# pranshu-raj-211/dmdqn

Hardware: NVIDIA B200
Metric: agent-updates/sec (higher is better)
Workload: dtype f32

## Files before the change

dmdqn_b200/csrc/learn_tc.cu:

```cuda
#include <cuda.h>
#include <string.h>
#include "common.cuh"

namespace dmdqn {

namespace {

constexpr int H = 256;
constexpr int BM = 128;
constexpr int EW = 16;
constexpr int NT = EW * 32;
constexpr int W_MMA = EW, W_TMA = EW + 1, W_CONV = EW + 2;
constexpr int CONV_WARPS = 6, CONV_GROUP_WARPS = 2;
constexpr int NT_F = (EW + 8) * 32;
constexpr int REGS_EPI = 104, REGS_AUX = 32;
constexpr int KC = 16;
constexpr uint32_t ATOM = BM * 128;
constexpr unsigned long long WAIT_LIMIT_NS = 2000000000ull;

__device__ __forceinline__ uint32_t smem_u32(const void* p) { return (uint32_t)__cvta_generic_to_shared(p); }

__device__ __forceinline__ uint64_t make_desc(uint32_t saddr, uint32_t lbo_bytes, uint32_t sbo_bytes, uint32_t layout) {
    return (uint64_t)((saddr >> 4) & 0x3FFF) | (uint64_t)((lbo_bytes >> 4) & 0x3FFF) << 16 |
           (uint64_t)((sbo_bytes >> 4) & 0x3FFF) << 32 | (uint64_t)1 << 46 | (uint64_t)layout << 61;
// ... 59 lines not shown
template <int N> __device__ __forceinline__ void regs_inc() { asm volatile("setmaxnreg.inc.sync.aligned.u32 %0;" ::"n"(N)); }
template <int N> __device__ __forceinline__ void regs_dec() { asm volatile("setmaxnreg.dec.sync.aligned.u32 %0;" ::"n"(N)); }
__device__ __forceinline__ void epi_sync() { asm volatile("bar.sync 1, 512;" ::: "memory"); }
__device__ __forceinline__ void l2_prefetch(const void* p, uint32_t bytes) {
    asm volatile("cp.async.bulk.prefetch.L2.global [%0], %1;" ::"l"(p), "r"(bytes) : "memory");
}
__device__ __forceinline__ void fence_async_smem() { asm volatile("fence.proxy.async.shared::cta;" ::: "memory"); }
__device__ __forceinline__ void tc_fence_before() { asm volatile("tcgen05.fence::before_thread_sync;" ::: "memory"); }
__device__ __forceinline__ void tc_fence_after() { asm volatile("tcgen05.fence::after_thread_sync;" ::: "memory"); }

__device__ __forceinline__ void tmem_ld32(uint32_t taddr, float (&v)[32]) {
    uint32_t r[32];
    asm volatile(
        "tcgen05.ld.sync.aligned.32x32b.x32.b32 {%0,%1,%2,%3,%4,%5,%6,%7,%8,%9,%10,%11,%12,%13,%14,%15,%16,%17,%18,%19,%20,%21,"
        "%22,%23,%24,%25,%26,%27,%28,%29,%30,%31}, [%32];\n"
        : "=r"(r[0]), "=r"(r[1]), "=r"(r[2]), "=r"(r[3]), "=r"(r[4]), "=r"(r[5]), "=r"(r[6]), "=r"(r[7]), "=r"(r[8]),
          "=r"(r[9]), "=r"(r[10]), "=r"(r[11]), "=r"(r[12]), "=r"(r[13]), "=r"(r[14]), "=r"(r[15]), "=r"(r[16]),
          "=r"(r[17]), "=r"(r[18]), "=r"(r[19]), "=r"(r[20]), "=r"(r[21]), "=r"(r[22]), "=r"(r[23]), "=r"(r[24]),
          "=r"(r[25]), "=r"(r[26]), "=r"(r[27]), "=r"(r[28]), "=r"(r[29]), "=r"(r[30]), "=r"(r[31])
        : "r"(taddr));
    asm volatile("tcgen05.wait::ld.sync.aligned;" ::: "memory");
#pragma unroll
    for (int j = 0; j < 32; ++j) v[j] = __uint_as_float(r[j]);
}
__device__ __forceinline__ void tmem_st32(uint32_t taddr, const float (&v)[32]) {
    asm volatile(
        "tcgen05.st.sync.aligned.32x32b.x32.b32 [%0], {%1,%2,%3,%4,%5,%6,%7,%8,%9,%10,%11,%12,%13,%14,%15,%16,%17,%18,%19,%20,"
        "%21,%22,%23,%24,%25,%26,%27,%28,%29,%30,%31,%32};\n" ::"r"(taddr),
        "r"(__float_as_uint(v[0])), "r"(__float_as_uint(v[1])), "r"(__float_as_uint(v[2])), "r"(__float_as_uint(v[3])),
        "r"(__float_as_uint(v[4])), "r"(__float_as_uint(v[5])), "r"(__float_as_uint(v[6])), "r"(__float_as_uint(v[7])),
        "r"(__float_as_uint(v[8])), "r"(__float_as_uint(v[9])), "r"(__float_as_uint(v[10])), "r"(__float_as_uint(v[11])),
        "r"(__float_as_uint(v[12])), "r"(__float_as_uint(v[13])), "r"(__float_as_uint(v[14])), "r"(__float_as_uint(v[15])),
        "r"(__float_as_uint(v[16])), "r"(__float_as_uint(v[17])), "r"(__float_as_uint(v[18])), "r"(__float_as_uint(v[19])),
        "r"(__float_as_uint(v[20])), "r"(__float_as_uint(v[21])), "r"(__float_as_uint(v[22])), "r"(__float_as_uint(v[23])),
        "r"(__float_as_uint(v[24])), "r"(__float_as_uint(v[25])), "r"(__float_as_uint(v[26])), "r"(__float_as_uint(v[27])),
        "r"(__float_as_uint(v[28])), "r"(__float_as_uint(v[29])), "r"(__float_as_uint(v[30])), "r"(__float_as_uint(v[31]))
        : "memory");
}
__device__ __forceinline__ void tmem_st_wait() { asm volatile("tcgen05.wait::st.sync.aligned;" ::: "memory"); }

__device__ __forceinline__ float tf32_hi(float x) {
    return __uint_as_float((__float_as_uint(x) + 0x1000u) & 0xffffe000u);
}
template <int PASSES>
__device__ __forceinline__ void split4(const float4& x, float4& hi, float4& lo) {
    if (PASSES == 1) { hi = x; lo = make_float4(0.f, 0.f, 0.f, 0.f); return; }
    hi = make_float4(tf32_hi(x.x), tf32_hi(x.y), tf32_hi(x.z), tf32_hi(x.w));
    lo = make_float4(x.x - hi.x, x.y - hi.y, x.z - hi.z, x.w - hi.w);
}

__device__ __forceinline__ uint32_t off_k128(int rows, int r, int k) {
    return (uint32_t)((k >> 5) * rows * 128 + r * 128 + ((((k & 31) >> 2) ^ (r & 7)) << 4) + ((k & 3) << 2));
}
__device__ __forceinline__ uint32_t off_mn(int mn_total, int k, int mn) {
    return (uint32_t)((k >> 2) * (mn_total >> 5) * 512 + (mn >> 5) * 512 + (k & 3) * 128 +
                      ((((mn & 31) >> 3) ^ (k & 3)) << 5) + ((mn & 7) << 2));
}

__device__ __forceinline__ void flag_release_add(int* f) {
    asm volatile("red.release.gpu.global.add.s32 [%0], 1;" ::"l"(f) : "memory");
}
__device__ __forceinline__ bool flag_acquire_ge(const int* f, int want) {
    for (int i = 0; i < (1 << 21); ++i) {
        int v;
        asm volatile("ld.acquire.gpu.global.s32 %0, [%1];" : "=r"(v) : "l"(f) : "memory");
        if (v >= want) return true;
        __nanosleep(256);
    }
    return false;
}
#ifdef TC_TIMING
__device__ __forceinline__ unsigned smid_() { unsigned r; asm volatile("mov.u32 %0, %%smid;" : "=r"(r)); return r; }
#endif
__device__ __forceinline__ void pdl_launch_dependents() { asm volatile("griddepcontrol.launch_dependents;" ::: "memory"); }

#ifdef TC_TIMING
#define KT_BEGIN const long long kt0_ = clock64(); long long kt1_ = 0
#define KT_END(name) do { if (threadIdx.x == 0 && (blockIdx.x % 37 == 0 || blockIdx.x == gridDim.x - 1)) \
        printf("%s cta %d kernel total %lld cycles, first item at %lld\n", name, blockIdx.x, clock64() - kt0_, kt1_ - kt0_); } while (0)
#define KT_FIRST() do { if (!kt1_) kt1_ = clock64(); } while (0)
#define TS_DECL long long ts_[16]; int tsi_ = 0
#define TS() do { if (tsi_ < 16) ts_[tsi_++] = clock64(); } while (0)
#define TS_D(i) (i < tsi_ ? ts_[i] - ts_[i - 1] : 0LL)
#define TS_PRINT(name) do { if (TC_TIMING > 1 && threadIdx.x == 0 && (blockIdx.x == 0 || blockIdx.x == 77 || blockIdx.x == gridDim.x - 1)) \
        printf("%s cta %d: %lld %lld %lld %lld %lld %lld %lld %lld %lld %lld %lld %lld | total %lld\n", name, blockIdx.x, TS_D(1), TS_D(2), TS_D(3), \
               TS_D(4), TS_D(5), TS_D(6), TS_D(7), TS_D(8), TS_D(9), TS_D(10), TS_D(11), TS_D(12), ts_[tsi_ - 1] - ts_[0]); tsi_ = 0; } while (0)
#define WG_TS_DECL long long wts_[20]; int wtsi_ = 0
#define WG_TS() do { if (wtsi_ < 20) wts_[wtsi_++] = clock64(); } while (0)
#define WG_D(i) ((i) < wtsi_ ? wts_[i] - wts_[(i) - 1] : 0LL)
#define WG_TS_PRINT(name, cond) do { if (TC_TIMING > 1 && (cond) && (blockIdx.x == 0 || blockIdx.x == 100)) \
        printf("%s cta %d: %lld %lld %lld %lld %lld %lld %lld %lld %lld %lld %lld %lld %lld %lld\n", name, blockIdx.x, WG_D(1), WG_D(2), WG_D(3), WG_D(4), \
               WG_D(5), WG_D(6), WG_D(7), WG_D(8), WG_D(9), WG_D(10), WG_D(11), WG_D(12), WG_D(13), WG_D(14)); } while (0)
#else
#define KT_FIRST()
#define KT_BEGIN
#define KT_END(name)
#define TS_DECL
#define TS()
#define TS_PRINT(name)
#define WG_TS_DECL
#define WG_TS()
#define WG_TS_PRINT(name, cond)
#endif

struct Fwd {
    static constexpr uint32_t R = 0;
    static constexpr uint32_t XLO = 3 * ATOM;
    static constexpr uint32_t WB = 8 * ATOM;
    static constexpr uint32_t BIAS1 = WB + 81920;
    static constexpr uint32_t BIAS2 = BIAS1 + 1024;
    static constexpr uint32_t W3S = BIAS2 + 1024;
    static constexpr uint32_t QP = W3S + 4096;
    static constexpr uint32_t ROWF = QP + 8192;
    static constexpr uint32_t BARS = ROWF + 3840;
    static constexpr uint32_t TOTAL = ROWF + 4096;
};
struct Bar {
    static constexpr uint32_t TMA_B = 112, CONV_B = 152, EMPTY_B = 192;
    static constexpr uint32_t AREADY = 232, DONE = 240;
    static constexpr uint32_t TMEM = 248;
};
constexpr int NSB = 5;
constexpr uint32_t STG_B = 16384, RAW_B = 8192;

struct Ring {
    uint32_t b = 0, gemms = 0;
};

__device__ __forceinline__ float4 ldg_stream(const float* p) {
    float4 v;
    asm volatile("ld.global.nc.L1::no_allocate.v4.f32 {%0,%1,%2,%3}, [%4];" : "=f"(v.x), "=f"(v.y), "=f"(v.z), "=f"(v.w) : "l"(p));
    return v;
}
__device__ __forceinline__ float4 ldg_plain(const float* p) {
    float4 v;
    asm volatile("ld.global.cg.v4.f32 {%0,%1,%2,%3}, [%4];" : "=f"(v.x), "=f"(v.y), "=f"(v.z), "=f"(v.w) : "l"(p));
    return v;
}
__device__ __forceinline__ void sts4(uint32_t a, const float4& v) {
    asm volatile("st.shared.v4.f32 [%0], {%1,%2,%3,%4};" ::"r"(a), "f"(v.x), "f"(v.y), "f"(v.z), "f"(v.w) : "memory");
}
__device__ __forceinline__ float4 lds4(uint32_t a) {
    float4 v;
    asm volatile("ld.shared.v4.f32 {%0,%1,%2,%3}, [%4];" : "=f"(v.x), "=f"(v.y), "=f"(v.z), "=f"(v.w) : "r"(a));
    return v;
}

constexpr int PF = 6;
__device__ __forceinline__ bool tma_fwd(uint32_t sbase, const CUtensorMap* tm, int g, const float* __restrict__ W, int K, Ring& r,
                                            bool ok, const float* __restrict__ next) {
    const uint32_t bars = sbase + Fwd::BARS;
    const int nchunks = K >> 3;
    for (int c = 0; c < nchunks; ++c) {
        const uint32_t s = r.b % NSB, u = r.b / NSB;
        if (c + PF < nchunks) l2_prefetch(W + (size_t)(c + PF) * 8 * H, RAW_B);
        else if (next) l2_prefetch(next + (size_t)(c + PF - nchunks) * 8 * H, RAW_B);
        if (u && ok) ok = mbar_wait(bars + Bar::EMPTY_B + 8 * s, (u - 1) & 1);
        mbar_expect_tx(bars + Bar::TMA_B + 8 * s, RAW_B);
        tma_load_5d(sbase + Fwd::WB + s * STG_B, tm, 0, 0, 0, 2 * c, g, bars + Bar::TMA_B + 8 * s);
        ++r.b;
    }
    return ok;
}
__device__ __forceinline__ bool tma_bwd(uint32_t sbase, const CUtensorMap* tm, int g, Ring& r, bool ok) {
    const uint32_t bars = sbase + Fwd::BARS;
    for (int c = 0; c < H / 8; ++c) {
        const uint32_t s = r.b % NSB, u = r.b / NSB;
        if (u && ok) ok = mbar_wait(bars + Bar::EMPTY_B + 8 * s, (u - 1) & 1);
        mbar_expect_tx(bars + Bar::TMA_B + 8 * s, RAW_B);
        tma_load_3d(sbase + Fwd::WB + s * STG_B, tm, c * 8, 0, g, bars + Bar::TMA_B + 8 * s);
        ++r.b;
    }
    return ok;
}
template <int PASSES>
__device__ __forceinline__ bool conv_ring(uint32_t sbase, int grp, int t, Ring& r, bool ok, int nchunks = H / 8) {
    const uint32_t bars = sbase + Fwd::BARS;
    constexpr int NGRP = CONV_WARPS / CONV_GROUP_WARPS;
    for (int c = 0; c < nchunks; ++c) {
        const uint32_t b = r.b + (uint32_t)c;
        if ((int)(b % NGRP) != grp) continue;
        const uint32_t s = b % NSB, u = b / NSB;
        const uint32_t st = sbase + Fwd::WB + s * STG_B;
        if (u && ok) ok = mbar_wait(bars + Bar::CONV_B + 8 * s, (u - 1) & 1);
        if (ok) ok = mbar_wait(bars + Bar::TMA_B + 8 * s, u & 1);
#pragma unroll
        for (int half = 0; half < 2; ++half) {
            float4 x[4];
#pragma unroll
            for (int i = 0; i < 4; ++i) x[i] = lds4(st + (uint32_t)(t + 64 * (4 * half + i)) * 16u);
#pragma unroll
            for (int i = 0; i < 4; ++i) {
                float4 hi, lo;
                split4<PASSES>(x[i], hi, lo);
                const uint32_t o = st + (uint32_t)(t + 64 * (4 * half + i)) * 16u;
                if (PASSES == 3) { sts4(o, hi); sts4(o + RAW_B, lo); }
            }
        }
        fence_async_smem();
        __syncwarp();
        if ((threadIdx.x & 31) == 0) mbar_arrive(bars + Bar::CONV_B + 8 * s);
    }
    r.b += (uint32_t)nchunks;
    return ok;
}

template <int PASSES, bool BT>
__device__ __forceinline__ bool mma_gemm(uint32_t sbase, uint32_t tmem, uint32_t a_hi, uint32_t a_lo_smem, uint32_t a_lo_tmem,
                                         int K, Ring& r, bool ok) {
    const uint32_t bars = sbase + Fwd::BARS;
    constexpr int KCX = 8;
    constexpr uint32_t idesc = make_idesc(false, !BT);
    const uint64_t a_hi0 = make_desc(a_hi, 16, 1024, 2);
    const uint64_t a_lo0 = make_desc(a_lo_smem, 16, 1024, 2);
    const uint64_t b0 = BT ? make_desc(sbase + Fwd::WB, 16, 256, 6) : make_desc(sbase + Fwd::WB, 512, 4096, 1);
    if (ok) ok = mbar_wait(bars + Bar::AREADY, r.gemms & 1);
    tc_fence_after();
    const int nchunks = K / KCX;
    for (int c = 0; c < nchunks; ++c) {
        const uint32_t s = r.b % NSB, u = r.b / NSB;
        if (ok) ok = mbar_wait(bars + Bar::CONV_B + 8 * s, u & 1);
        tc_fence_after();
#pragma unroll
        for (int ks = 0; ks < KCX / 8; ++ks) {
            const int kg = c * KCX + ks * 8;
            const uint32_t a_off = ((uint32_t)(kg >> 5) * ATOM + (uint32_t)((kg & 31) >> 3) * 32) >> 4;
            const uint32_t b_off = (s * STG_B) >> 4;
            const uint64_t a_hi_d = a_hi0 + a_off;
            const uint64_t b_hi = b0 + b_off, b_lo = b0 + b_off + (RAW_B >> 4);
            uint32_t acc = (c | ks) ? 1u : 0u;
            if (PASSES == 3) {
                if (a_lo_smem) mma_ss(tmem, a_lo0 + a_off, b_hi, idesc, acc);
                else mma_ts(tmem, a_lo_tmem + (uint32_t)kg, b_hi, idesc, acc);
                mma_ss(tmem, a_hi_d, b_lo, idesc, 1u);
                acc = 1u;
            }
            mma_ss(tmem, a_hi_d, b_hi, idesc, acc);
        }
        umma_commit(bars + Bar::EMPTY_B + 8 * s);
        ++r.b;
    }
    umma_commit(bars + Bar::DONE);
    r.gemms += 1;
    return ok;
}

__device__ __forceinline__ void a_ready(uint32_t sbase) {
    fence_async_smem();
    tc_fence_before();
    __syncwarp();
    if ((threadIdx.x & 31) == 0) mbar_arrive(sbase + Fwd::BARS + Bar::AREADY);
}
__device__ __forceinline__ bool wait_gemm(uint32_t sbase, Ring& r, bool ok) {
    if (ok) ok = mbar_wait(sbase + Fwd::BARS + Bar::DONE, r.gemms & 1);
    tc_fence_after();
    r.gemms += 1;
    return ok;
}

template <int PASSES>
struct XGather {
    static constexpr int MAXP = BM * 96 / 4 / NT;
    float4 x[MAXP];
    uint32_t off[MAXP];
    int n;
    float4 sp;

    __device__ __forceinline__ void begin(const float* __restrict__ ring, const int32_t* __restrict__ rows, int r0, int B, int Dp,
                                          const float* __restrict__ P, const float* __restrict__ W3, const Layout& L) {
        {
            const int j = threadIdx.x;
            if (j < H) { sp.x = __ldg(P + L.b1 + j); sp.y = __ldg(P + L.b2 + j); }
            else sp = __ldg(reinterpret_cast<const float4*>(W3) + (j - H));
        }
        const int q = Dp >> 2;
        n = BM * q / NT;
        const int dr = NT / q, dp = NT % q;
        int r = threadIdx.x / q, pc = threadIdx.x % q;
        int32_t rid[MAXP], col[MAXP];
#pragma unroll
        for (int j = 0; j < MAXP; ++j) {
            rid[j] = -1;
            if (j < n) {
                if (r0 + r < B) rid[j] = __ldg(rows + r0 + r);
                off[j] = off_k128(BM, r, pc << 2);
                col[j] = pc << 2;
                r += dr; pc += dp;
                if (pc >= q) { pc -= q; r += 1; }
            }
        }
#pragma unroll
        for (int j = 0; j < MAXP; ++j) {
            x[j] = make_float4(0.f, 0.f, 0.f, 0.f);
            if (j < n && rid[j] >= 0) x[j] = ldg_stream(ring + (size_t)rid[j] * Dp + col[j]);
        }
    }
    __device__ __forceinline__ void store(uint32_t sbase) {
        {
            float* s = reinterpret_cast<float*>(__cvta_shared_to_generic((size_t)sbase));
            const int j = threadIdx.x;
            if (j < H) { s[Fwd::BIAS1 / 4 + j] = sp.x; s[Fwd::BIAS2 / 4 + j] = sp.y; }
            else reinterpret_cast<float4*>(s + Fwd::W3S / 4)[j - H] = sp;
        }
#pragma unroll
        for (int j = 0; j < MAXP; ++j) {
            if (j < n) {
                float4 hi, lo;
                split4<PASSES>(x[j], hi, lo);
                sts4(sbase + Fwd::R + off[j], hi);
                if (PASSES == 3) sts4(sbase + Fwd::XLO + off[j], lo);
            }
        }
    }
};

struct Epi {
    int row, part;
    uint32_t lane_addr;
    __device__ __forceinline__ Epi() {
        const int warp = threadIdx.x >> 5, lane = threadIdx.x & 31;
        row = (warp & 3) * 32 + lane;
        part = warp >> 2;
        lane_addr = (uint32_t)((warp & 3) * 32) << 16;
    }
};

template <int PASSES>
__device__ __forceinline__ void epi_hidden(uint32_t sbase, uint32_t tmem, const Epi& e, uint32_t bias_off,
                                           float* __restrict__ gout_t, int ldt, uint32_t (&mask)[2]) {
#pragma unroll 1
    for (int cc = 0; cc < 2; ++cc) {
        const int c0 = e.part * 64 + cc * 32;
        float v[32], lo[32];
        float4 bq[8];
#pragma unroll
        for (int j = 0; j < 8; ++j)
            bq[j] = lds4(sbase + bias_off + (uint32_t)(c0 + 4 * j) * 4);
        tmem_ld32(tmem + e.lane_addr + (uint32_t)c0, v);
        uint32_t m = 0;
#pragma unroll
        for (int j = 0; j < 32; j += 4) {
            const float4 b = bq[j >> 2];
            float4 x = make_float4(fmaxf(v[j] + b.x, 0.f), fmaxf(v[j + 1] + b.y, 0.f), fmaxf(v[j + 2] + b.z, 0.f),
                                   fmaxf(v[j + 3] + b.w, 0.f));
            m |= (x.x > 0.f ? 1u : 0u) << j | (x.y > 0.f ? 1u : 0u) << (j + 1) | (x.z > 0.f ? 1u : 0u) << (j + 2) |
                 (x.w > 0.f ? 1u : 0u) << (j + 3);
            if (gout_t) {
                gout_t[(size_t)(c0 + j) * ldt] = x.x; gout_t[(size_t)(c0 + j + 1) * ldt] = x.y;
                gout_t[(size_t)(c0 + j + 2) * ldt] = x.z; gout_t[(size_t)(c0 + j + 3) * ldt] = x.w;
            }
            float4 hi, l4;
            split4<PASSES>(x, hi, l4);
            sts4(sbase + Fwd::R + off_k128(BM, e.row, c0 + j), hi);
            lo[j] = l4.x; lo[j + 1] = l4.y; lo[j + 2] = l4.z; lo[j + 3] = l4.w;
        }
        mask[cc] = m;
        if (PASSES == 3) tmem_st32(tmem + e.lane_addr + 256u + (uint32_t)c0, lo);
    }
    if (PASSES == 3) tmem_st_wait();
}

__device__ __forceinline__ void epi_head(uint32_t sbase, uint32_t tmem, const Epi& e, bool keep_h2,
                                         uint32_t (&mask)[2], float (&q)[4], const float* __restrict__ b3) {
    float4 acc = make_float4(0.f, 0.f, 0.f, 0.f);
#pragma unroll 1
    for (int cc = 0; cc < 2; ++cc) {
        const int c0 = e.part * 64 + cc * 32;
        float v[32];
        tmem_ld32(tmem + e.lane_addr + (uint32_t)c0, v);
        uint32_t m = 0;
#pragma unroll
        for (int j = 0; j < 32; ++j) {
            float b;
            asm volatile("ld.shared.f32 %0, [%1];" : "=f"(b) : "r"(sbase + Fwd::BIAS2 + (uint32_t)(c0 + j) * 4));
            const float x = fmaxf(v[j] + b, 0.f);
            v[j] = x;
            m |= (x > 0.f ? 1u : 0u) << j;
            const float4 w = lds4(sbase + Fwd::W3S + (uint32_t)(c0 + j) * 16);
            acc.x = fmaf(x, w.x, acc.x); acc.y = fmaf(x, w.y, acc.y);
            acc.z = fmaf(x, w.z, acc.z); acc.w = fmaf(x, w.w, acc.w);
        }
        mask[cc] = m;
        if (keep_h2) {
#pragma unroll
            for (int j = 0; j < 32; j += 4)
                sts4(sbase + Fwd::R + off_k128(BM, e.row, c0 + j), make_float4(v[j], v[j + 1], v[j + 2], v[j + 3]));
        }
    }
    float4* qp = reinterpret_cast<float4*>(__cvta_shared_to_generic((size_t)(sbase + Fwd::QP)));
    qp[e.part * BM + e.row] = acc;
    epi_sync();
    const float4 p0 = qp[e.row], p1 = qp[BM + e.row], p2 = qp[2 * BM + e.row], p3 = qp[3 * BM + e.row];
    q[0] = ((p0.x + p1.x) + (p2.x + p3.x)) + __ldg(b3 + 0); q[1] = ((p0.y + p1.y) + (p2.y + p3.y)) + __ldg(b3 + 1);
    q[2] = ((p0.z + p1.z) + (p2.z + p3.z)) + __ldg(b3 + 2); q[3] = ((p0.w + p1.w) + (p2.w + p3.w)) + __ldg(b3 + 3);
}

__device__ __forceinline__ uint32_t tc_prologue(uint32_t sbase) {
    const int warp = threadIdx.x >> 5;
    const uint32_t bars = sbase + Fwd::BARS;
    if (threadIdx.x == 0) {
        for (int b = 0; b < NSB; ++b) {
            mbar_init(bars + Bar::TMA_B + 8 * b, 1);
            mbar_init(bars + Bar::CONV_B + 8 * b, CONV_GROUP_WARPS);
            mbar_init(bars + Bar::EMPTY_B + 8 * b, 1);
        }
        mbar_init(bars + Bar::AREADY, EW);
        mbar_init(bars + Bar::DONE, 1);
        asm volatile("fence.mbarrier_init.release.cluster;" ::: "memory");
    }
    if (warp == 0) {
        asm volatile("tcgen05.alloc.cta_group::1.sync.aligned.shared::cta.b32 [%0], %1;" ::"r"(bars + Bar::TMEM), "r"(512));
        asm volatile("tcgen05.relinquish_alloc_permit.cta_group::1.sync.aligned;" ::);
    }
    tc_fence_before();
    __syncthreads();
    tc_fence_after();
    uint32_t tmem;
    asm volatile("ld.shared.u32 %0, [%1];" : "=r"(tmem) : "r"(bars + Bar::TMEM));
    return tmem;
}
__device__ __forceinline__ void tc_epilogue(uint32_t tmem) {
    tc_fence_before();
    __syncthreads();
    if ((threadIdx.x >> 5) == 0) asm volatile("tcgen05.dealloc.cta_group::1.sync.aligned.b32 %0, %1;" ::"r"(tmem), "r"(512));
}

template <bool DUELING>
__device__ __forceinline__ const float* head_w3(const LearnArgs& A, const float* P, int tgt, int g) {
    if constexpr (DUELING) return (tgt ? A.head[1] : A.head[0]) + (size_t)g * A.head_stride;
    else return P + A.L.w3;
}
template <bool DUELING>
__device__ __forceinline__ const float* head_b3(const LearnArgs& A, const float* P, int tgt, int g) {
    if constexpr (DUELING) return head_w3<true>(A, P, tgt, g) + 4 * H;
    else return P + A.L.b3;
}

__device__ __forceinline__ int k3_next(const LearnArgs& A, int q, int n_items) {
    while (q < n_items && !A.active[(q >> 1) / A.tc_tiles]) q += gridDim.x;
    return q;
}

template <int PASSES, bool DUELING>
__global__ void __launch_bounds__(NT_F, 1) tc_target_kernel(const LearnArgs A, const __grid_constant__ CUtensorMap tm_w1,
                                                            const __grid_constant__ CUtensorMap tm_w2,
                                                            const __grid_constant__ CUtensorMap tm_w1t,
                                                            const __grid_constant__ CUtensorMap tm_w2t) {
    extern __shared__ uint8_t smem_raw[];
    const uint32_t sbase = (smem_u32(smem_raw) + 1023u) & ~1023u;
    const int B = A.d.batch, Dp = A.d.obs_stride;
    const int n_items = 2 * A.d.n_nets * A.tc_tiles;
    const int warp = threadIdx.x >> 5;
    KT_BEGIN;
    const uint32_t tmem = tc_prologue(sbase);
    if (A.chain) {
        asm volatile("griddepcontrol.wait;" ::: "memory");
        pdl_launch_dependents();
    }
    Ring ring;
    bool ok = true;
    if (warp >= EW) {
        regs_dec<REGS_AUX>();
      if (warp == W_MMA) {
        if ((threadIdx.x & 31) == 0) {
            int prev = -1;
            for (int q = k3_next(A, blockIdx.x, n_items); q < n_items; q = k3_next(A, q + gridDim.x, n_items)) {
                ok = mma_gemm<PASSES, false>(sbase, tmem, sbase + Fwd::R, sbase + Fwd::XLO, 0, Dp, ring, ok);
                if (prev >= 0) flag_release_add(A.k3_done + (size_t)((prev >> 1) / A.tc_tiles) * A.ws_tiles + (prev >> 1) % A.tc_tiles);
                prev = q;
                ok = mma_gemm<PASSES, false>(sbase, tmem, sbase + Fwd::R, 0, tmem + 256u, H, ring, ok);
            }
            if (!ok) atomicExch(A.error, 13);
        }
        __syncwarp();
      } else if (warp == W_TMA) {
        if ((threadIdx.x & 31) == 0) {
            for (int q = k3_next(A, blockIdx.x, n_items); q < n_items;) {
                const int g = (q >> 1) / A.tc_tiles;
                const float* P = ((q & 1) ? A.nets.theta_tgt : A.nets.theta) + (size_t)g * A.L.stride;
                const int qn = k3_next(A, q + gridDim.x, n_items);
                const float* Pn = qn < n_items ? ((qn & 1) ? A.nets.theta_tgt : A.nets.theta) + (size_t)((qn >> 1) / A.tc_tiles) * A.L.stride + A.L.w1 : nullptr;
                ok = tma_fwd(sbase, (q & 1) ? &tm_w1t : &tm_w1, g, P + A.L.w1, Dp, ring, ok, P + A.L.w2);
                ok = tma_fwd(sbase, (q & 1) ? &tm_w2t : &tm_w2, g, P + A.L.w2, H, ring, ok, Pn);
                q = qn;
            }
            if (!ok) atomicExch(A.error, 23);
        }
        __syncwarp();
      } else if (warp < W_CONV + CONV_WARPS) {
        const int tc = threadIdx.x - W_CONV * 32, cg = (warp - W_CONV) / CONV_GROUP_WARPS, t = tc % (CONV_GROUP_WARPS * 32);
        for (int q = k3_next(A, blockIdx.x, n_items); q < n_items; q = k3_next(A, q + gridDim.x, n_items)) {
            ok = conv_ring<PASSES>(sbase, cg, t, ring, ok, Dp / 8);
            ok = conv_ring<PASSES>(sbase, cg, t, ring, ok, H / 8);
        }
        if (!ok && tc == 0) atomicExch(A.error, 33);
      }
    } else {
        regs_inc<REGS_EPI>();
        const Epi e;
        XGather<PASSES> xg;
        int q = k3_next(A, blockIdx.x, n_items);
        if (q < n_items) {
            const int g = (q >> 1) / A.tc_tiles, rt = (q >> 1) % A.tc_tiles;
            const float* P = ((q & 1) ? A.nets.theta_tgt : A.nets.theta) + (size_t)g * A.L.stride;
            xg.begin(A.rp.next_obs, A.nrows + (size_t)g * B, rt * BM, B, Dp, P, head_w3<DUELING>(A, P, q & 1, g), A.L);
        }
        int q_last = -1;
        while (q < n_items) {
            const int item = q >> 1, pass = q & 1;
            const int g = item / A.tc_tiles, rt = item % A.tc_tiles, r0 = rt * BM;
            const float* P = (pass == 0 ? A.nets.theta : A.nets.theta_tgt) + (size_t)g * A.L.stride;
            TS_DECL;
            TS();
            KT_FIRST();
            xg.store(sbase);
            a_ready(sbase);
            epi_sync();
            TS();
            ok = wait_gemm(sbase, ring, ok);
            TS();
            uint32_t mask[2];
            epi_hidden<PASSES>(sbase, tmem, e, Fwd::BIAS1, nullptr, 0, mask);
            a_ready(sbase);
            TS();
            const int qn = k3_next(A, q + gridDim.x, n_items);
            if (qn < n_items) {
                const int gn = (qn >> 1) / A.tc_tiles, rtn = (qn >> 1) % A.tc_tiles;
                const float* Pn = ((qn & 1) ? A.nets.theta_tgt : A.nets.theta) + (size_t)gn * A.L.stride;
                xg.begin(A.rp.next_obs, A.nrows + (size_t)gn * B, rtn * BM, B, Dp, Pn, head_w3<DUELING>(A, Pn, qn & 1, gn), A.L);
            }
            ok = wait_gemm(sbase, ring, ok);
            TS();
            float qv[4];
            epi_head(sbase, tmem, e, false, mask, qv, head_b3<DUELING>(A, P, pass, g));
            TS();
            TS_PRINT("K3 store L1 epi1 L2 epi2");
            const int gr = r0 + e.row;
            if (e.part == 0 && gr < B) {
                float* out = (pass == 0 ? A.q_next : A.tq_all) + ((size_t)g * B + gr) * 4;
                *reinterpret_cast<float4*>(out) = make_float4(qv[0], qv[1], qv[2], qv[3]);
            }
            q_last = q;
            q = qn;
        }
        epi_sync();
        if (q_last >= 0 && threadIdx.x == 0) flag_release_add(A.k3_done + (size_t)((q_last >> 1) / A.tc_tiles) * A.ws_tiles + (q_last >> 1) % A.tc_tiles);
        if (!ok && threadIdx.x == 0) atomicExch(A.error, 3);
        KT_END("K3");
    }
    tc_epilogue(tmem);
}

__device__ __forceinline__ int k4_next(const LearnArgs& A, int q, int n_items) {
    while (q < n_items && !A.active[q / A.tc_tiles]) q += gridDim.x;
    return q;
}

template <int PASSES, bool DUELING>
__global__ void __launch_bounds__(NT_F, 1) tc_online_kernel(const LearnArgs A, const __grid_constant__ CUtensorMap tmap_w2,
                                                            const __grid_constant__ CUtensorMap tm_w1,
                                                            const __grid_constant__ CUtensorMap tm_w2) {
    extern __shared__ uint8_t smem_raw[];
    const uint32_t sbase = (smem_u32(smem_raw) + 1023u) & ~1023u;
    float* sf = reinterpret_cast<float*>(__cvta_shared_to_generic((size_t)sbase));
    const int B = A.d.batch, Dp = A.d.obs_stride;
    const int n_items = A.d.n_nets * A.tc_tiles;
    const int warp = threadIdx.x >> 5;
    KT_BEGIN;
    const uint32_t tmem = tc_prologue(sbase);
    if (A.chain) pdl_launch_dependents();
    Ring ring;
    bool ok = true;
    if (warp >= EW) {
        regs_dec<REGS_AUX>();
      if (warp == W_MMA) {
        if ((threadIdx.x & 31) == 0) {
            int prev = -1;
            for (int q = k4_next(A, blockIdx.x, n_items); q < n_items; q = k4_next(A, q + gridDim.x, n_items)) {
                ok = mma_gemm<PASSES, false>(sbase, tmem, sbase + Fwd::R, sbase + Fwd::XLO, 0, Dp, ring, ok);
                ok = mma_gemm<PASSES, false>(sbase, tmem, sbase + Fwd::R, 0, tmem + 256u, H, ring, ok);
                if (prev >= 0) flag_release_add(A.k4a_done + prev / A.tc_tiles);
                prev = q;
                ok = mma_gemm<PASSES, true>(sbase, tmem, sbase + Fwd::R, 0, tmem + 256u, H, ring, ok);
            }
            if (!ok) atomicExch(A.error, 14);
        }
        __syncwarp();
      } else if (warp == W_TMA) {
        if ((threadIdx.x & 31) == 0) {
            for (int q = k4_next(A, blockIdx.x, n_items); q < n_items; q = k4_next(A, q + gridDim.x, n_items)) {
                const int g = q / A.tc_tiles;
                if (A.chain && ok) ok = flag_acquire_ge(A.k3_done + (size_t)g * A.ws_tiles + q % A.tc_tiles, 2);
                const float* P = A.nets.theta + (size_t)g * A.L.stride;
                const int qn = k4_next(A, q + gridDim.x, n_items);
                const float* Pn = qn < n_items ? A.nets.theta + (size_t)(qn / A.tc_tiles) * A.L.stride + A.L.w1 : nullptr;
                ok = tma_fwd(sbase, &tm_w1, g, P + A.L.w1, Dp, ring, ok, P + A.L.w2);
                ok = tma_fwd(sbase, &tm_w2, g, P + A.L.w2, H, ring, ok, Pn);
                ok = tma_bwd(sbase, &tmap_w2, g, ring, ok);
            }
            if (!ok) atomicExch(A.error, 24);
        }
        __syncwarp();
      } else if (warp < W_CONV + CONV_WARPS) {
        const int tc = threadIdx.x - W_CONV * 32, cg = (warp - W_CONV) / CONV_GROUP_WARPS, t = tc % (CONV_GROUP_WARPS * 32);
        for (int q = k4_next(A, blockIdx.x, n_items); q < n_items; q = k4_next(A, q + gridDim.x, n_items)) {
            ok = conv_ring<PASSES>(sbase, cg, t, ring, ok, Dp / 8);
            ok = conv_ring<PASSES>(sbase, cg, t, ring, ok, H / 8);
            ok = conv_ring<PASSES>(sbase, cg, t, ring, ok, H / 8);
        }
        if (!ok && tc == 0) atomicExch(A.error, 34);
      }
    } else {
        regs_inc<REGS_EPI>();
        const Epi e;
        XGather<PASSES> xg;
        int q = k4_next(A, blockIdx.x, n_items);
        if (q < n_items) {
            const float* P = A.nets.theta + (size_t)(q / A.tc_tiles) * A.L.stride;
            xg.begin(A.rp.obs, A.rows + (size_t)(q / A.tc_tiles) * B, (q % A.tc_tiles) * BM, B, Dp, P, head_w3<DUELING>(A, P, 0, q / A.tc_tiles), A.L);
        }
        int q_last = -1;
        while (q < n_items) {
            const int g = q / A.tc_tiles, rt = q % A.tc_tiles, r0 = rt * BM;
            const size_t sb = (size_t)g * B;
            const float* P = A.nets.theta + (size_t)g * A.L.stride;
            const int gr = r0 + e.row;
            const bool valid = gr < B;
            TS_DECL;
            TS();
            KT_FIRST();
            if (q_last < 0) {
                xg.store(sbase);
                a_ready(sbase);
            }
            epi_sync();
            TS();
            ok = wait_gemm(sbase, ring, ok);
            TS();
            uint32_t mask1[2], mask2[2];
            epi_hidden<PASSES>(sbase, tmem, e, Fwd::BIAS1, valid ? A.h1 + sb * H + gr : nullptr, B, mask1);
            a_ready(sbase);
            TS();
            float yi = 0.f;
            if (valid) {
                const float4 qo = ldg_plain(A.q_next + (sb + gr) * 4);
                const float4 qt = ldg_plain(A.tq_all + (sb + gr) * 4);
                const float q_on[4] = {qo.x, qo.y, qo.z, qo.w}, q_tg[4] = {qt.x, qt.y, qt.z, qt.w};
                float bmax = q_on[0], tq = q_tg[0], tmax = q_tg[0];
#pragma unroll
                for (int k = 1; k < 4; ++k) {
                    if (k < A.d.n_actions) {
                        if (q_on[k] > bmax) { bmax = q_on[k]; tq = q_tg[k]; }
                        tmax = fmaxf(tmax, q_tg[k]);
                    }
                }
                tq = A.double_dqn ? tq : tmax;
                yi = A.r_hat[sb + gr] + A.disc_b[sb + gr] * tq;
                if (e.part == 0) A.y[sb + gr] = yi;
            }
            const int ai_pre = valid ? A.act_b[sb + gr] : 0;
            ok = wait_gemm(sbase, ring, ok);
            TS();
            float qv[4];
            epi_head(sbase, tmem, e, true, mask2, qv, head_b3<DUELING>(A, P, 0, g));
            TS();

            float gi = 0.f, term = 0.f;
            int ai = 0;
            if (valid) {
                ai = ai_pre;
                const float qa = ai == 0 ? qv[0] : ai == 1 ? qv[1] : ai == 2 ? qv[2] : qv[3];
                const float err = qa - yi;
                if (A.loss == DMDQN_LOSS_MSE) {
                    term = err * err;
                    gi = (2.0f * err) / (float)A.loss_batch;
                } else {
                    const float ae = fabsf(err);
                    term = ae <= 1.0f ? 0.5f * err * err : ae - 0.5f;
                    gi = fminf(fmaxf(err, -1.0f), 1.0f) / (float)A.loss_batch;
                }
                if (A.per) {
                    const float wi = A.is_w[sb + gr];
                    term = wi * term;
                    gi = wi * gi;
                    if (e.part == 0 && ok) per_store_priority(A, A.rows[sb + gr], err);
                }
                if (e.part == 0) {
                    A.ga[sb + gr] = make_float2(gi, __int_as_float(ai));
                    *reinterpret_cast<float4*>(A.q_all + (sb + gr) * 4) = make_float4(qv[0], qv[1], qv[2], qv[3]);
                }
            }
            float* rowf = sf + Fwd::ROWF / 4;
            if (e.part == 0) {
                reinterpret_cast<float4*>(rowf + BM)[e.row] = make_float4(ai == 0 ? gi : 0.f, ai == 1 ? gi : 0.f, ai == 2 ? gi : 0.f, ai == 3 ? gi : 0.f);
                float red[11];
                red[0] = term;
                red[1] = 0.f; red[2] = 0.f;
#pragma unroll
                for (int k = 0; k < 4; ++k) {
                    const float qq = (valid && k < A.d.n_actions) ? qv[k] : 0.f;
                    red[1] += qq;
                    red[2] = fmaf(qq, qq, red[2]);
                    red[3 + k] = (valid && ai == k) ? 1.f : 0.f;
                    red[7 + k] = (valid && ai == k) ? gi : 0.f;
                }
#pragma unroll
                for (int o = 16; o > 0; o >>= 1)
#pragma unroll
                    for (int v = 0; v < 11; ++v) red[v] += __shfl_xor_sync(0xffffffffu, red[v], o);
                if ((threadIdx.x & 31) == 0)
#pragma unroll
                    for (int v = 0; v < 11; ++v) rowf[7 * BM + (threadIdx.x >> 5) * 11 + v] = red[v];
            }
            epi_sync();
            TS();
            if (threadIdx.x < 11) {
                const float* wp = rowf + 7 * BM + threadIdx.x;
                const float tot = ((wp[0] + wp[11]) + wp[22]) + wp[33];
                const size_t pt = (size_t)g * A.tc_tiles + rt;
                if (threadIdx.x < 7) A.part_loss[pt * 8 + threadIdx.x] = tot;
                else A.part_b3[pt * 4 + (threadIdx.x - 7)] = tot;
            }
            {
                const int w = threadIdx.x >> 5, l = threadIdx.x & 31;
                const int j0 = ((w & 7) * 8 + (l & 7)) * 4, rh = w >> 3, rg = l >> 3;
                float4 w3c[4];
#pragma unroll
                for (int c = 0; c < 4; ++c) w3c[c] = lds4(sbase + Fwd::W3S + (uint32_t)(j0 + c) * 16);
                float d[4][4], s2[4];
#pragma unroll
                for (int c = 0; c < 4; ++c) { d[c][0] = d[c][1] = d[c][2] = d[c][3] = 0.f; s2[c] = 0.f; }
                const uint32_t hrow = sbase + Fwd::R + (uint32_t)(j0 >> 5) * ATOM;
                const uint32_t piece = (uint32_t)((j0 & 31) >> 2);
                const uint32_t gsel = sbase + Fwd::ROWF + BM * 4;
                const int i_begin = rh * (BM / 2) + rg * 16;
#pragma unroll 4
                for (int u = 0; u < 16; ++u) {
                    const int i = i_begin + u;
                    const float4 h4 = lds4(hrow + (uint32_t)i * 128u + ((piece ^ (uint32_t)(i & 7)) << 4));
                    const float4 gs = lds4(gsel + (uint32_t)i * 16u);
                    const float hv[4] = {h4.x, h4.y, h4.z, h4.w};
#pragma unroll
                    for (int c = 0; c < 4; ++c) {
                        d[c][0] = fmaf(hv[c], gs.x, d[c][0]); d[c][1] = fmaf(hv[c], gs.y, d[c][1]);
                        d[c][2] = fmaf(hv[c], gs.z, d[c][2]); d[c][3] = fmaf(hv[c], gs.w, d[c][3]);
                        const float gw = fmaf(gs.w, w3c[c].w, fmaf(gs.z, w3c[c].z, fmaf(gs.y, w3c[c].y, gs.x * w3c[c].x)));
                        s2[c] += hv[c] > 0.f ? gw : 0.f;
                    }
                }
#pragma unroll
                for (int o = 8; o <= 16; o <<= 1) {
#pragma unroll
                    for (int c = 0; c < 4; ++c) {
#pragma unroll
                        for (int a = 0; a < 4; ++a) d[c][a] += __shfl_xor_sync(0xffffffffu, d[c][a], o);
                        s2[c] += __shfl_xor_sync(0xffffffffu, s2[c], o);
                    }
                }
                TS();
                float* up = sf + Fwd::QP / 4;
                if (rh == 1 && rg == 0) {
#pragma unroll
                    for (int c = 0; c < 4; ++c) {
                        reinterpret_cast<float4*>(up)[(j0 + c) * 2] = make_float4(d[c][0], d[c][1], d[c][2], d[c][3]);
                        up[(j0 + c) * 8 + 4] = s2[c];
                    }
                }
                epi_sync();
                if (rh == 0 && rg == 0) {
                    const size_t pt = (size_t)g * A.tc_tiles + rt;
                    float sb2[4];
#pragma unroll
                    for (int c = 0; c < 4; ++c) {
                        const float4 u4 = reinterpret_cast<const float4*>(up)[(j0 + c) * 2];
                        reinterpret_cast<float4*>(A.part_w3 + pt * H * 4)[j0 + c] = make_float4(d[c][0] + u4.x, d[c][1] + u4.y, d[c][2] + u4.z, d[c][3] + u4.w);
                        sb2[c] = s2[c] + up[(j0 + c) * 8 + 4];
                    }
                    *reinterpret_cast<float4*>(A.part_b2 + pt * H + j0) = make_float4(sb2[0], sb2[1], sb2[2], sb2[3]);
                }
            }
            epi_sync();
            TS();

            if (valid) reinterpret_cast<uint2*>(A.mask2)[(sb + gr) * 4 + e.part] = make_uint2(mask2[0], mask2[1]);
            if (rt == 0 && threadIdx.x < H)
                reinterpret_cast<float4*>(A.w3_copy + (size_t)g * H * 4)[threadIdx.x] =
                    *reinterpret_cast<const float4*>(sf + Fwd::W3S / 4 + threadIdx.x * 4);
#pragma unroll 1
            for (int cc = 0; cc < 2; ++cc) {
                const int c0 = e.part * 64 + cc * 32;
                float lo[32], wv[32];
#pragma unroll
                for (int j = 0; j < 32; ++j)
                    asm volatile("ld.shared.f32 %0, [%1];" : "=f"(wv[j]) : "r"(sbase + Fwd::W3S + (uint32_t)(c0 + j) * 16 + (uint32_t)ai * 4));
#pragma unroll
                for (int j = 0; j < 32; j += 4) {
                    float x[4];
#pragma unroll
                    for (int t = 0; t < 4; ++t) x[t] = ((mask2[cc] >> (j + t)) & 1u) ? gi * wv[j + t] : 0.f;
                    float4 hi, l4;
                    split4<PASSES>(make_float4(x[0], x[1], x[2], x[3]), hi, l4);
                    sts4(sbase + Fwd::R + off_k128(BM, e.row, c0 + j), hi);
                    lo[j] = l4.x; lo[j + 1] = l4.y; lo[j + 2] = l4.z; lo[j + 3] = l4.w;
                }
                if (PASSES == 3) tmem_st32(tmem + e.lane_addr + 256u + (uint32_t)c0, lo);
            }
            if (PASSES == 3) tmem_st_wait();
            a_ready(sbase);
            TS();
            const int qn = k4_next(A, q + gridDim.x, n_items);
            if (qn < n_items) {
                const float* Pn = A.nets.theta + (size_t)(qn / A.tc_tiles) * A.L.stride;
                xg.begin(A.rp.obs, A.rows + (size_t)(qn / A.tc_tiles) * B, (qn % A.tc_tiles) * BM, B, Dp, Pn, head_w3<DUELING>(A, Pn, 0, qn / A.tc_tiles),
                         A.L);
            }
            ok = wait_gemm(sbase, ring, ok);
            TS();
            {
                float v[32];
                const int c0 = e.part * 64;
                tmem_ld32(tmem + e.lane_addr + (uint32_t)c0, v);
                if (valid) {
#pragma unroll
                    for (int j = 0; j < 32; ++j)
                        A.dh1[sb * H + (size_t)(c0 + j) * B + gr] = ((mask1[0] >> j) & 1u) ? v[j] : 0.f;
                }
                tmem_ld32(tmem + e.lane_addr + (uint32_t)(c0 + 32), v);
                if (qn < n_items) {
                    xg.store(sbase);
                    a_ready(sbase);
                }
                if (valid) {
#pragma unroll
                    for (int j = 0; j < 32; ++j)
                        A.dh1[sb * H + (size_t)(c0 + 32 + j) * B + gr] = ((mask1[1] >> j) & 1u) ? v[j] : 0.f;
                }
            }
            TS();
            TS_PRINT("K4a store L1 epi1 L2 epi2 loss dW3loop dW3out dh2 bwdGEMM dh1store");
            q_last = q;
            q = qn;
        }
        epi_sync();
        if (q_last >= 0 && threadIdx.x == 0) flag_release_add(A.k4a_done + q_last / A.tc_tiles);
        if (!ok && threadIdx.x == 0) atomicExch(A.error, 4);
        KT_END("K4a");
    }
    tc_epilogue(tmem);
}

__device__ __forceinline__ void adam1(const AdamStep& k, float g, float& th, float& m, float& v, float& tg) {
    m = m + (g - m) * k.one_m_b1;
    v = v + (g * g - v) * k.one_m_b2;
    float sq;
    asm("sqrt.approx.f32 %0, %1;" : "=f"(sq) : "f"(v));
    th = th - __fdividef(m * k.alpha, sq + k.eps);
    if (k.sync == 1) tg = th;
    else if (k.sync == 2) tg = k.tau * th + (1.0f - k.tau) * tg;
}

__device__ __forceinline__ void adam_fast(const AdamStep& k, float g, float& th, float& m, float& v) {
    m = m + (g - m) * k.one_m_b1;
    v = v + (g * g - v) * k.one_m_b2;
    float sq;
    asm("sqrt.approx.f32 %0, %1;" : "=f"(sq) : "f"(v));
    th = th - __fdividef(m * k.alpha, sq + k.eps);
}

struct Wg {
    static constexpr int STAGES = 3;
    static constexpr uint32_t A_BYTES = KC * BM * 4;
    static constexpr uint32_t B_BYTES = KC * H * 4;
    static constexpr uint32_t AUX = 2 * A_BYTES + 2 * B_BYTES;
    static constexpr uint32_t AUX_MASK = 128;
    static constexpr uint32_t AUX_BYTES = 6144;
    static constexpr uint32_t STG = AUX + AUX_BYTES;
    static constexpr int TLD = 36;
    static constexpr uint32_t TILES = STAGES * STG;
    static constexpr uint32_t W3T = TILES + 8 * 32 * TLD * 4;
    static constexpr uint32_t BARS = W3T + 2 * 4 * H * 4;
    static constexpr uint32_t FULL = 0, CONV = 24, EMPTY = 48, ACC_FULL = 72, ACC_FREE = 88, TMEM = 104;
    static constexpr int NQ = 8;
    static constexpr uint32_t QFULL = 112, QITEM = QFULL + 8 * NQ;
    static constexpr uint32_t TOTAL = BARS + 256;
    static constexpr int EPI_WARPS = 8, CONV_WARPS = 8;
    static constexpr int NCONV = CONV_WARPS * 32;
    static constexpr int NTW = 20 * 32;
    static constexpr int REGS_EPI = 160, REGS_CONV = 64, REGS_AUX = 32;
};
__device__ __forceinline__ void conv_sync() { asm volatile("bar.sync 1, 256;" ::: "memory"); }

__device__ __forceinline__ void wg_item(int q, int G, int& g, int& t) {
    if (q < 2 * G) { g = q >> 1; t = q & 1; }
    else { g = q - 2 * G; t = 2; }
}

__device__ __forceinline__ int wg_pop(uint32_t bars, int& nq, bool& ok) {
    const uint32_t slot = (uint32_t)nq & (Wg::NQ - 1);
    int q = -1;
    if ((threadIdx.x & 31) == 0) {
        if (ok) ok = mbar_wait(bars + Wg::QFULL + 8 * slot, (uint32_t)(nq >> 3) & 1u);
        if (ok) asm volatile("ld.shared.s32 %0, [%1];" : "=r"(q) : "r"(bars + Wg::QITEM + 4 * slot));
    }
    ++nq;
    q = __shfl_sync(0xffffffffu, q, 0);
    if (q < 0) ok = __shfl_sync(0xffffffffu, (int)ok, 0) != 0;
    return q;
}
__device__ __forceinline__ float ldcg_f(const float* p) {
    float v;
    asm volatile("ld.global.cg.f32 %0, [%1];" : "=f"(v) : "l"(p));
    return v;
}

template <int PASSES>
__global__ void __launch_bounds__(Wg::NTW, 1) tc_wgrad_kernel(const LearnArgs A, const __grid_constant__ CUtensorMap tmap_h1,
                                                              const __grid_constant__ CUtensorMap tmap_dh1) {
    extern __shared__ uint8_t smem_raw[];
    const int B = A.d.batch, Dp = A.d.obs_stride, G = A.d.n_nets;
    const int tid = threadIdx.x, warp = tid >> 5, lane = tid & 31;
    const uint32_t sbase = (smem_u32(smem_raw) + 1023u) & ~1023u;
    const uint32_t bars = sbase + Wg::BARS;
    const int n_items = 3 * G;
    const int nchunks = (B + KC - 1) / KC;

    if (tid == 0) {
        for (int s = 0; s < Wg::STAGES; ++s) {
            mbar_init(bars + Wg::FULL + 8 * s, 1);
            mbar_init(bars + Wg::CONV + 8 * s, Wg::CONV_WARPS);
            mbar_init(bars + Wg::EMPTY + 8 * s, 1);
        }
        for (int b = 0; b < 2; ++b) {
            mbar_init(bars + Wg::ACC_FULL + 8 * b, 1);
            mbar_init(bars + Wg::ACC_FREE + 8 * b, Wg::EPI_WARPS);
        }
        for (int b = 0; b < Wg::NQ; ++b) mbar_init(bars + Wg::QFULL + 8 * b, 1);
        asm volatile("fence.mbarrier_init.release.cluster;" ::: "memory");
    }
    if (warp == 0) {
        asm volatile("tcgen05.alloc.cta_group::1.sync.aligned.shared::cta.b32 [%0], %1;" ::"r"(bars + Wg::TMEM), "r"(512));
        asm volatile("tcgen05.relinquish_alloc_permit.cta_group::1.sync.aligned;" ::);
    }
    tc_fence_before();
// ... 517 lines not shown
```

Baseline: 541,500.

## Double-buffer TMEM accumulators in K3 and stage next tile's inputs before head epilogue

The K3 target/online forward kernel now alternates between two TMEM accumulator halves per work item, with the other half holding the low-precision split. The epilogue warps write the next item's X rows and bias1 into shared memory and signal A-ready before running the current head epilogue, while bias2/W3 are stored separately at the top of the loop. The aim is to let the MMA warp start the next item's first GEMM while the epilogue is still reading the previous accumulator. This relies on the TMEM and shared-memory regions not being overwritten while still in use, and the split of bias1 and bias2/W3 stores adds ordering risk.

Result: faster. 547,500, median of 6 (+1.1%).

```diff
diff --git a/dmdqn_b200/csrc/learn_tc.cu b/dmdqn_b200/csrc/learn_tc.cu
--- a/dmdqn_b200/csrc/learn_tc.cu
+++ b/dmdqn_b200/csrc/learn_tc.cu
@@ -385,6 +385,20 @@
             if (j < H) { s[Fwd::BIAS1 / 4 + j] = sp.x; s[Fwd::BIAS2 / 4 + j] = sp.y; }
             else reinterpret_cast<float4*>(s + Fwd::W3S / 4)[j - H] = sp;
         }
+        store_x(sbase);
+    }
+    __device__ __forceinline__ void store_rows(uint32_t sbase) {
+        float* s = reinterpret_cast<float*>(__cvta_shared_to_generic((size_t)sbase));
+        if (threadIdx.x < H) s[Fwd::BIAS1 / 4 + threadIdx.x] = sp.x;
+        store_x(sbase);
+    }
+    __device__ __forceinline__ void store_head(uint32_t sbase) {
+        float* s = reinterpret_cast<float*>(__cvta_shared_to_generic((size_t)sbase));
+        const int j = threadIdx.x;
+        if (j < H) s[Fwd::BIAS2 / 4 + j] = sp.y;
+        else reinterpret_cast<float4*>(s + Fwd::W3S / 4)[j - H] = sp;
+    }
+    __device__ __forceinline__ void store_x(uint32_t sbase) {
 #pragma unroll
         for (int j = 0; j < MAXP; ++j) {
             if (j < n) {
@@ -409,7 +423,7 @@
 };
 
 template <int PASSES>
-__device__ __forceinline__ void epi_hidden(uint32_t sbase, uint32_t tmem, const Epi& e, uint32_t bias_off,
+__device__ __forceinline__ void epi_hidden(uint32_t sbase, uint32_t tmem, uint32_t tmem_lo, const Epi& e, uint32_t bias_off,
                                            float* __restrict__ gout_t, int ldt, uint32_t (&mask)[2]) {
 #pragma unroll 1
     for (int cc = 0; cc < 2; ++cc) {
@@ -438,7 +452,7 @@
             lo[j] = l4.x; lo[j + 1] = l4.y; lo[j + 2] = l4.z; lo[j + 3] = l4.w;
         }
         mask[cc] = m;
-        if (PASSES == 3) tmem_st32(tmem + e.lane_addr + 256u + (uint32_t)c0, lo);
+        if (PASSES == 3) tmem_st32(tmem_lo + e.lane_addr + (uint32_t)c0, lo);
     }
     if (PASSES == 3) tmem_st_wait();
 }
@@ -547,11 +561,13 @@
       if (warp == W_MMA) {
         if ((threadIdx.x & 31) == 0) {
             int prev = -1;
-            for (int q = k3_next(A, blockIdx.x, n_items); q < n_items; q = k3_next(A, q + gridDim.x, n_items)) {
-                ok = mma_gemm<PASSES, false>(sbase, tmem, sbase + Fwd::R, sbase + Fwd::XLO, 0, Dp, ring, ok);
+            uint32_t k = 0;
+            for (int q = k3_next(A, blockIdx.x, n_items); q < n_items; q = k3_next(A, q + gridDim.x, n_items), ++k) {
+                const uint32_t acc = tmem + ((k & 1u) << 8), lo = acc ^ 256u;
+                ok = mma_gemm<PASSES, false>(sbase, acc, sbase + Fwd::R, sbase + Fwd::XLO, 0, Dp, ring, ok);
+                ok = mma_gemm<PASSES, false>(sbase, acc, sbase + Fwd::R, 0, lo, H, ring, ok);
                 if (prev >= 0) flag_release_add(A.k3_done + (size_t)((prev >> 1) / A.tc_tiles) * A.ws_tiles + (prev >> 1) % A.tc_tiles);
                 prev = q;
-                ok = mma_gemm<PASSES, false>(sbase, tmem, sbase + Fwd::R, 0, tmem + 256u, H, ring, ok);
             }
             if (!ok) atomicExch(A.error, 13);
         }
@@ -587,23 +603,26 @@
             const int g = (q >> 1) / A.tc_tiles, rt = (q >> 1) % A.tc_tiles;
             const float* P = ((q & 1) ? A.nets.theta_tgt : A.nets.theta) + (size_t)g * A.L.stride;
             xg.begin(A.rp.next_obs, A.nrows + (size_t)g * B, rt * BM, B, Dp, P, head_w3<DUELING>(A, P, q & 1, g), A.L);
+            xg.store_rows(sbase);
+            a_ready(sbase);
         }
         int q_last = -1;
+        uint32_t k = 0;
         while (q < n_items) {
             const int item = q >> 1, pass = q & 1;
             const int g = item / A.tc_tiles, rt = item % A.tc_tiles, r0 = rt * BM;
             const float* P = (pass == 0 ? A.nets.theta : A.nets.theta_tgt) + (size_t)g * A.L.stride;
+            const uint32_t acc = tmem + ((k & 1u) << 8), lo = acc ^ 256u;
             TS_DECL;
             TS();
             KT_FIRST();
-            xg.store(sbase);
-            a_ready(sbase);
+            xg.store_head(sbase);
             epi_sync();
             TS();
             ok = wait_gemm(sbase, ring, ok);
             TS();
             uint32_t mask[2];
-            epi_hidden<PASSES>(sbase, tmem, e, Fwd::BIAS1, nullptr, 0, mask);
+            epi_hidden<PASSES>(sbase, acc, lo, e, Fwd::BIAS1, nullptr, 0, mask);
             a_ready(sbase);
             TS();
             const int qn = k3_next(A, q + gridDim.x, n_items);
@@ -614,10 +633,15 @@
             }
             ok = wait_gemm(sbase, ring, ok);
             TS();
+            if (qn < n_items) {
+                xg.store_rows(sbase);
+                a_ready(sbase);
+            }
+            TS();
             float qv[4];
-            epi_head(sbase, tmem, e, false, mask, qv, head_b3<DUELING>(A, P, pass, g));
-            TS();
-            TS_PRINT("K3 store L1 epi1 L2 epi2");
+            epi_head(sbase, acc, e, false, mask, qv, head_b3<DUELING>(A, P, pass, g));
+            TS();
+            TS_PRINT("K3 b2W3 L1 epi1 L2 store epi2");
             const int gr = r0 + e.row;
             if (e.part == 0 && gr < B) {
                 float* out = (pass == 0 ? A.q_next : A.tq_all) + ((size_t)g * B + gr) * 4;
@@ -625,6 +649,7 @@
             }
             q_last = q;
             q = qn;
+            ++k;
         }
         epi_sync();
         if (q_last >= 0 && threadIdx.x == 0) flag_release_add(A.k3_done + (size_t)((q_last >> 1) / A.tc_tiles) * A.ws_tiles + (q_last >> 1) % A.tc_tiles);
@@ -721,7 +746,7 @@
             ok = wait_gemm(sbase, ring, ok);
             TS();
             uint32_t mask1[2], mask2[2];
-            epi_hidden<PASSES>(sbase, tmem, e, Fwd::BIAS1, valid ? A.h1 + sb * H + gr : nullptr, B, mask1);
+            epi_hidden<PASSES>(sbase, tmem, tmem + 256u, e, Fwd::BIAS1, valid ? A.h1 + sb * H + gr : nullptr, B, mask1);
             a_ready(sbase);
             TS();
             float yi = 0.f;
```
